# CarloLucibello/GraphNeuralNetworks.jl

Measured on AMD Instinct MI355X. Metric: edges/sec (fwd) GCNConv+GATConv, ogbn-products-shape; achieved HBM GB/s vs peak, higher is better.
Workload: dtype f32; 1 GPU; products-shape power-law graph N=2449029 E=61859140 (+N self loops, E'=64308169), D=100: GCNConv(100=>100,relu) fwd + GATConv(100=>16,heads=8,relu) fwd per step; edges counted = 2*E' per GPU; parallelism=replicas x1 (independent feature batches, no collective)

## Files before the change

graphneuralnetworks.jl_amd/csrc/plan.hip:

```cpp
#include <cstring>
#include <algorithm>
#include <vector>

#include "common.h"
#include "launch.h"
#include "pool.h"
#include "scratch.h"
#include "sort_scan.h"

namespace gnnmp {

int ensure_workspace(gnnmp_graph *p, size_t floats) { return grow(p->ws, p->ws_floats, floats, "hipMalloc(plan workspace)"); }

int ensure_arrive(gnnmp_graph *p, size_t n, size_t floats, hipStream_t stream) {
    GNNMP_TRY(grow(p->spart, p->spart_floats, floats, "hipMalloc(plan slice partials)"));
    if (n <= p->arrive_n) return GNNMP_OK;
    GNNMP_TRY(grow(p->arrive, p->arrive_n, n, "hipMalloc(plan arrival counters)"));
    const hipError_t e = hipMemsetAsync(p->arrive, 0, sizeof(uint32_t) * n, stream);
    if (e != hipSuccess) {
        p->arrive_n = 0;
        return hip_fail(e, "hipMemsetAsync(plan arrival counters)");
    }
    return GNNMP_OK;
}
// ... 88 lines not shown
    if (!ok) *bad = 1;
    rowptr[i] = (uint32_t)(ok ? v : (i == n_dst ? E : 0));
}
__global__ void csc_col_kernel(const void *rowval, int idx_bytes, int base, int64_t E, int64_t n_src, int32_t *col, int32_t *eid, int *bad) {
    int64_t p = (int64_t)blockIdx.x * blockDim.x + threadIdx.x;
    if (p >= E) return;
    int64_t s = load_index(rowval, p, idx_bytes, base);
    if (s < 0 || s >= n_src) {
        *bad = 1;
        s = 0;
    }
    col[p] = (int32_t)s;
    eid[p] = (int32_t)(uint32_t)p;
}

__global__ void plan_long_rows(const uint32_t *rowptr, int64_t n_dst, int thresh, int64_t *list,
                               int cap, int *count, unsigned long long *maxdeg) {
    int64_t i = (int64_t)blockIdx.x * blockDim.x + threadIdx.x;
    if (i >= n_dst) return;
    const int64_t beg = rowptr[i], end = rowptr[i + 1];
    const int64_t len = end - beg;
    if (len > 0) atomicMax(maxdeg, (unsigned long long)len);
    if (len > thresh) {
        int pos = atomicAdd(count, 1);
        if (pos < cap) {
            list[3 * pos] = i;
            list[3 * pos + 1] = beg;
            list[3 * pos + 2] = end;
        }
    }
}
__global__ void widen_u32_kernel(const uint32_t *in, int64_t n, int64_t *out) {
    int64_t i = (int64_t)blockIdx.x * blockDim.x + threadIdx.x;
    if (i < n) out[i] = (int64_t)in[i];
}

__global__ void slot_gather_kernel(const int32_t *idx, const float *v, int64_t Etot, int64_t n_valid,
                                   float *out) {
    int64_t p = (int64_t)blockIdx.x * blockDim.x + threadIdx.x;
    if (p >= Etot) return;
    const int64_t k = (uint32_t)idx[p];
    out[p] = k < n_valid ? v[k] : 1.0f;
}

__global__ void self_loops_kernel(const void *src, const void *dst, int idx_bytes, int base,
// ... 47 lines not shown

static inline unsigned nblocks(int64_t n, int bs) { return (unsigned)((n + bs - 1) / bs); }

int plan_long_thresh(int64_t Etot) {
    if (knob(KNOB_LONG_ROW) > 0) return knob(KNOB_LONG_ROW);
    int th = GNNMP_MIN_LONG_ROW;
    while (th < GNNMP_LONG_ROW && (double)th < 4e-5 * (double)Etot) th <<= 1;
    return th;
}

static int plan_chunk_slots() {
    const int v = knob(KNOB_CHUNK_SLOTS);
    return v >= 16 ? v : 128;
}

int plan_build_long_rows(gnnmp_graph *p, hipStream_t stream) {
    const int64_t n_dst = p->n_dst, Etot = p->n_total;
    const int BS = 256;
    const int cap = (int)std::min<int64_t>(Etot / std::max(1, p->long_thresh) + 1, n_dst + 1);
    DevBuf<int64_t> long_tmp;
    DevBuf<int> flags;
    GNNMP_HIP(flags.alloc(4));
    GNNMP_HIP(hipMemsetAsync(flags.get(), 0, sizeof(int) * 4, stream));
    GNNMP_HIP(long_tmp.alloc(3 * (size_t)std::max(cap, 1)));
    if (n_dst > 0) {
        plan_long_rows<<<nblocks(n_dst, BS), BS, 0, stream>>>(p->rowptr, n_dst, p->long_thresh, long_tmp.get(), cap, flags.get(),
                                                              reinterpret_cast<unsigned long long *>(flags.get() + 2));
        GNNMP_HIP(hipGetLastError());
    }
    int meta[4] = {0, 0, 0, 0};
    GNNMP_HIP(hipMemcpyAsync(meta, flags.get(), sizeof(int) * 4, hipMemcpyDeviceToHost, stream));
    GNNMP_HIP(hipStreamSynchronize(stream));
    unsigned long long md;
    memcpy(&md, meta + 2, sizeof(md));
    p->max_degree = (int64_t)md;
    p->n_long = std::min(meta[0], cap);
    if (p->n_long == 0) return GNNMP_OK;
    struct Tri { int64_t row, beg, end; };
    std::vector<Tri> h((size_t)p->n_long);
    GNNMP_HIP(hipMemcpy(h.data(), long_tmp.get(), sizeof(Tri) * h.size(), hipMemcpyDeviceToHost));
    std::sort(h.begin(), h.end(), [](const Tri &a, const Tri &b) { return a.row < b.row; });
    std::vector<int32_t> rows, cptr, crow, clrow;
    std::vector<uint32_t> cbeg, cend;
    cptr.push_back(0);
    const int64_t clen = std::min<int64_t>(p->long_thresh, plan_chunk_slots());
    for (const Tri &t : h) {
        const int64_t len = t.end - t.beg;
        const int64_t nch = (len + clen - 1) / clen;
        const int64_t csz = (len + nch - 1) / nch;
        for (int64_t c = 0; c < nch; ++c) {
            crow.push_back((int32_t)t.row);
            clrow.push_back((int32_t)rows.size());
            cbeg.push_back((uint32_t)(t.beg + c * csz));
            cend.push_back((uint32_t)std::min(t.beg + (c + 1) * csz, t.end));
        }
        rows.push_back((int32_t)t.row);
        cptr.push_back((int32_t)crow.size());
    }
    if (crow.size() >= (size_t)INT32_MAX)
        return fail(GNNMP_EUNSUPPORTED, "plan_create: %zu chunks of split rows exceed the int32 chunk index", crow.size());
    p->n_chunks = (int)crow.size();
    auto upload = [&](auto *&dst, const auto &v) -> hipError_t {
        const size_t bytes = sizeof(v[0]) * v.size();
        const hipError_t e = alloc_into(dst, v.size());
        if (e != hipSuccess) return e;
        p->bytes += (int64_t)bytes;
        return hipMemcpy(dst, v.data(), bytes, hipMemcpyHostToDevice);
    };
    GNNMP_HIP(upload(p->long_rows, rows));
    GNNMP_HIP(upload(p->long_cptr, cptr));
    GNNMP_HIP(upload(p->chunk_row, crow));
    GNNMP_HIP(upload(p->chunk_lrow, clrow));
    GNNMP_HIP(upload(p->chunk_beg, cbeg));
    GNNMP_HIP(upload(p->chunk_end, cend));
    return GNNMP_OK;
}

}

using namespace gnnmp;

extern "C" {

int gnnmp_plan_destroy(gnnmp_graph_t *p) { return plan_dispose(p, nullptr, false); }

int gnnmp_plan_reset_counters(gnnmp_graph_t *p, gnnmp_stream_t stream_) {
    hipStream_t stream = (hipStream_t)stream_;
    if (!p) return fail(GNNMP_EINVAL, "plan_reset_counters: null plan");
    if (p->arrive && p->arrive_n) GNNMP_HIP(hipMemsetAsync(p->arrive, 0, sizeof(uint32_t) * p->arrive_n, stream));
    if (p->ticket) GNNMP_HIP(hipMemsetAsync(p->ticket, 0, 2 * sizeof(uint32_t), stream));
// ... 67 lines not shown
    const int64_t Etot = n_edges + (add_self_loops ? n_dst : 0);
    if (Etot >= (int64_t)GNNMP_MAX_SLOTS || n_src >= (int64_t)INT32_MAX || n_dst >= (int64_t)INT32_MAX)
        return fail(GNNMP_EUNSUPPORTED, "plan_create: E' = %lld (limit 2^32 - 65536) / N = %lld (limit 2^31 - 2) exceed the plan format",
                    (long long)Etot, (long long)std::max(n_src, n_dst));

    PlanPtr p(new gnnmp_graph_t());
    p->n_src = n_src;
    p->n_dst = n_dst;
    p->n_edges = n_edges;
    p->n_total = Etot;
    p->self_loops = add_self_loops ? 1 : 0;
    p->long_thresh = plan_long_thresh(Etot);

    const int BS = 256;
    const size_t epad = (size_t)std::max<int64_t>(Etot, 1);
    DevBuf<int> flags;
    DevBuf<unsigned char> sort_keys;
    uint32_t *keys_out = nullptr;
    GNNMP_HIP(alloc_into(p->rowptr, (size_t)(n_dst + 1)));
    GNNMP_HIP(alloc_into(p->col, epad));
    GNNMP_HIP(alloc_into(p->eid, epad));
    GNNMP_HIP(flags.alloc(4));
    GNNMP_HIP(hipMemsetAsync(flags.get(), 0, sizeof(int) * 4, stream));
    p->bytes = (int64_t)(sizeof(int32_t) * ((size_t)(n_dst + 1) + 2 * epad));

    if (Etot > 0) {
        const size_t piece = (sizeof(uint32_t) * epad + 255) & ~(size_t)255;
        GNNMP_HIP(sort_keys.alloc(3 * piece));
        uint32_t *keys_in = reinterpret_cast<uint32_t *>(sort_keys.get());
        keys_out = reinterpret_cast<uint32_t *>(sort_keys.get() + piece);
        uint32_t *vals_in = reinterpret_cast<uint32_t *>(sort_keys.get() + 2 * piece);
        plan_fill_keys<<<nblocks(Etot, BS), BS, 0, stream>>>(src, dst, idx_bytes, index_base,
                                                             n_edges, Etot, n_src, n_dst, keys_in,
                                                             vals_in, flags.get());
        GNNMP_HIP(hipGetLastError());
        if (validate) {
            int bad = 0;
            GNNMP_HIP(hipMemcpyAsync(&bad, flags.get(), sizeof(int), hipMemcpyDeviceToHost, stream));
            GNNMP_HIP(hipStreamSynchronize(stream));
            if (bad)
                return fail(GNNMP_EBOUNDS, "plan_create: edge index outside 1..N (n_src=%lld n_dst=%lld)",
                            (long long)n_src, (long long)n_dst);
        }
        unsigned bits = 1;
        while (bits < 32 && ((int64_t)1 << bits) < n_dst) ++bits;
        GNNMP_TRY(radix_sort_pairs_u32(keys_in, keys_out, vals_in, reinterpret_cast<uint32_t *>(p->eid), (size_t)Etot, 0, (int)bits,
                                       stream));
        plan_col<<<nblocks(Etot, BS), BS, 0, stream>>>(src, idx_bytes, index_base, n_edges, Etot,
                                                       reinterpret_cast<uint32_t *>(p->eid), p->col);
        GNNMP_HIP(hipGetLastError());
    }
    plan_rowptr<<<nblocks(n_dst + 1, BS), BS, 0, stream>>>(keys_out, Etot, n_dst, p->rowptr);
    GNNMP_HIP(hipGetLastError());

    GNNMP_TRY(plan_build_long_rows(p.get(), stream));
    *out = p.release();
    return GNNMP_OK;
}

int gnnmp_plan_from_csc(gnnmp_graph_t **out, const void *colptr, const void *rowval, int idx_bytes, int index_base, int64_t n_src,
                        int64_t n_dst, int64_t n_edges, int validate, gnnmp_stream_t stream_) {
    hipStream_t stream = (hipStream_t)stream_;
    if (!out) return fail(GNNMP_EINVAL, "plan_from_csc: out is NULL");
    *out = nullptr;
    if (idx_bytes != 4 && idx_bytes != 8) return fail(GNNMP_EINVAL, "plan_from_csc: idx_bytes must be 4 or 8 (got %d)", idx_bytes);
    if (index_base != 0 && index_base != 1) return fail(GNNMP_EINVAL, "plan_from_csc: index_base must be 0 or 1 (got %d)", index_base);
    if (n_src < 0 || n_dst < 0 || n_edges < 0) return fail(GNNMP_EINVAL, "plan_from_csc: negative size");
    if (!colptr || (n_edges > 0 && !rowval)) return fail(GNNMP_EINVAL, "plan_from_csc: null colptr / rowval");
    if (n_edges >= (int64_t)GNNMP_MAX_SLOTS || n_src >= (int64_t)INT32_MAX || n_dst >= (int64_t)INT32_MAX)
        return fail(GNNMP_EUNSUPPORTED, "plan_from_csc: E = %lld (limit 2^32 - 65536) / N = %lld (limit 2^31 - 2) exceed the plan format",
                    (long long)n_edges, (long long)std::max(n_src, n_dst));
    PlanPtr p(new gnnmp_graph_t());
    p->n_src = n_src;
    p->n_dst = n_dst;
    p->n_edges = n_edges;
    p->n_total = n_edges;
    p->long_thresh = plan_long_thresh(n_edges);
    const int BS = 256;
    const size_t epad = (size_t)std::max<int64_t>(n_edges, 1);
    DevBuf<int> flags;
    GNNMP_HIP(alloc_into(p->rowptr, (size_t)(n_dst + 1)));
    GNNMP_HIP(alloc_into(p->col, epad));
    GNNMP_HIP(alloc_into(p->eid, epad));
    GNNMP_HIP(flags.alloc(4));
    GNNMP_HIP(hipMemsetAsync(flags.get(), 0, sizeof(int) * 4, stream));
    p->bytes = (int64_t)(sizeof(int32_t) * ((size_t)(n_dst + 1) + 2 * epad));
    csc_rowptr_kernel<<<nblocks(n_dst + 1, BS), BS, 0, stream>>>(colptr, idx_bytes, index_base, n_dst, n_edges, p->rowptr, flags.get());
    GNNMP_HIP(hipGetLastError());
    if (n_edges > 0) {
        csc_col_kernel<<<nblocks(n_edges, BS), BS, 0, stream>>>(rowval, idx_bytes, index_base, n_edges, n_src, p->col, p->eid, flags.get());
        GNNMP_HIP(hipGetLastError());
    }
    (void)validate;
    int bad = 0;
    GNNMP_HIP(hipMemcpyAsync(&bad, flags.get(), sizeof(int), hipMemcpyDeviceToHost, stream));
    GNNMP_HIP(hipStreamSynchronize(stream));
    if (bad)
        return fail(GNNMP_EBOUNDS, "plan_from_csc: colptr is not a monotone 0..E column pointer, or a row index lies outside 1..n_src "
                    "(n_src=%lld n_dst=%lld E=%lld)", (long long)n_src, (long long)n_dst, (long long)n_edges);
    GNNMP_TRY(plan_build_long_rows(p.get(), stream));
    *out = p.release();
    return GNNMP_OK;
}

int gnnmp_plan_slot_gather_f32(gnnmp_graph_t *p, int by, const float *v, float *out_slot,
                               gnnmp_stream_t stream_) {
    hipStream_t stream = (hipStream_t)stream_;
    if (!p) return fail(GNNMP_EINVAL, "plan_slot_gather: null plan");
    if (by != 0 && by != 1) return fail(GNNMP_EINVAL, "plan_slot_gather: `by` must be 0 (node) or 1 (edge)");
    if (p->n_total == 0) return GNNMP_OK;
    if (!v || !out_slot) return fail(GNNMP_EINVAL, "plan_slot_gather: null pointer");
    if (by == 0)
        slot_gather_kernel<<<nblocks(p->n_total, 256), 256, 0, stream>>>(p->col, v, p->n_total, p->n_src, out_slot);
    else
        slot_gather_kernel<<<nblocks(p->n_total, 256), 256, 0, stream>>>(p->eid, v, p->n_total, p->n_edges, out_slot);
// ... 94 lines not shown
```

graphneuralnetworks.jl_amd/csrc/plan_edit.hip:

```cpp
#include <algorithm>

#include "common.h"
#include "launch.h"
#include "pool.h"
#include "sort_scan.h"

namespace gnnmp {
namespace {

constexpr int BS = 256;
inline unsigned nblk(int64_t n) { return (unsigned)std::max<int64_t>(1, (n + BS - 1) / BS); }
inline size_t up64(size_t n) { return (n + 63) & ~(size_t)63; }

struct PoolScratch {
    void *p = nullptr;
    size_t cap = 0;
    hipStream_t stream;
    explicit PoolScratch(hipStream_t s) : stream(s) {}
    PoolScratch(const PoolScratch &) = delete;
    PoolScratch &operator=(const PoolScratch &) = delete;
    ~PoolScratch() { pool_park(p, cap, stream, true); }
    bool take(size_t bytes) { return pool_take(&p, &cap, std::max<size_t>(bytes, 256), stream); }
};

__device__ __forceinline__ int64_t row_of_slot(const uint32_t *__restrict__ rowptr, int64_t n_rows, int64_t p) {
    int64_t lo = 0, hi = n_rows;
    while (hi - lo > 1) {
        const int64_t mid = (lo + hi) >> 1;
        if ((int64_t)rowptr[mid] <= p) lo = mid; else hi = mid;
    }
    return lo;
}

enum { META_NKEEP = 0, META_EKEEP = 1, META_SLOTS = 2, META_MAXDEG = 3, META_BAD = 4, META_WORDS = 8 };

__global__ void __launch_bounds__(BS) rm_mark_kernel(int64_t N, int random, int none, DropArgs d, uint32_t *__restrict__ keep) {
    const int64_t i = (int64_t)blockIdx.x * BS + threadIdx.x;
    if (i > N) return;
// ... 344 lines not shown
```

graphneuralnetworks.jl_amd/csrc/pool.h:

```cpp
#pragma once
#include <hip/hip_runtime.h>
#include <stddef.h>

namespace gnnmp {
bool pool_take(void **out, size_t *cap, size_t bytes, hipStream_t stream);
void pool_park(void *p, size_t cap, hipStream_t stream, bool stream_known);
int pool_pick(const size_t *caps, int n, size_t bytes);
void pool_trim();
}
```

graphneuralnetworks.jl_amd/csrc/pool.hip:

```cpp
#include <mutex>

#include "pool.h"
#include "common.h"

namespace gnnmp {
namespace {
struct Parked {
    void *p = nullptr;
    size_t cap = 0;
    hipStream_t stream = nullptr;
    hipEvent_t ev = nullptr;
};
constexpr int POOL_SLOTS = 8;
struct DevicePool {
    Parked slots[POOL_SLOTS];
    hipEvent_t free_events[POOL_SLOTS] = {};
    int n_free_events = 0;
};
DevicePool g_pools[GNNMP_MAX_DEVICES];
std::mutex g_lock;

hipEvent_t event_get(DevicePool &dp) {
    if (dp.n_free_events > 0) return dp.free_events[--dp.n_free_events];
    hipEvent_t e = nullptr;
    if (hipEventCreateWithFlags(&e, hipEventDisableTiming) != hipSuccess) return nullptr;
    return e;
}
void event_put(DevicePool &dp, hipEvent_t e) {
    if (!e) return;
    if (dp.n_free_events < POOL_SLOTS) dp.free_events[dp.n_free_events++] = e;
    else (void)hipEventDestroy(e);
}
bool same_stream(hipStream_t a, hipStream_t b) { return a == b && a != hipStreamPerThread; }
}

int pool_pick(const size_t *caps, int n, size_t bytes) {
    int best = -1;
    for (int i = 0; i < n; ++i)
        if (caps[i] && caps[i] >= bytes && (best < 0 || caps[i] < caps[best])) best = i;
    if (best >= 0 && caps[best] <= 2 * bytes + (1 << 20)) return best;
    return -1;
}

bool pool_take(void **out, size_t *cap, size_t bytes, hipStream_t stream) {
    DevicePool &dp = g_pools[current_device()];
    Parked got;
    {
        std::lock_guard<std::mutex> lk(g_lock);
        size_t caps[POOL_SLOTS];
        for (int i = 0; i < POOL_SLOTS; ++i) caps[i] = dp.slots[i].p ? dp.slots[i].cap : 0;
        const int best = pool_pick(caps, POOL_SLOTS, bytes);
        if (best >= 0) {
            got = dp.slots[best];
            dp.slots[best] = Parked();
        }
    }
    if (got.p) {
        bool ok = true;
        if (!got.ev) {
            ok = hipDeviceSynchronize() == hipSuccess;
// ... 1 lines not shown
            if (!same_stream(got.stream, stream)) ok = hipStreamWaitEvent(stream, got.ev, 0) == hipSuccess;
            std::lock_guard<std::mutex> lk(g_lock);
            event_put(dp, got.ev);
        }
        if (ok) {
            *out = got.p;
            *cap = got.cap;
            return true;
        }
        (void)hipFree(got.p);
    }
    *cap = bytes;
    return hipMalloc(out, bytes) == hipSuccess;
}

void pool_park(void *p, size_t cap, hipStream_t stream, bool stream_known) {
    if (!p) return;
    int dev = current_device();
    {
        hipPointerAttribute_t at;
        if (hipPointerGetAttributes(&at, p) == hipSuccess && at.device >= 0 && at.device < GNNMP_MAX_DEVICES) {
            if (at.device != dev) stream_known = false;
            dev = at.device;
        } else {
            (void)hipGetLastError();
        }
    }
    DevicePool &dp = g_pools[dev];
    Parked in;
    in.p = p;
    in.cap = cap;
    Parked evict;
    {
        std::lock_guard<std::mutex> lk(g_lock);
        if (stream_known) {
            in.stream = stream;
            in.ev = event_get(dp);
            if (in.ev && hipEventRecord(in.ev, stream) != hipSuccess) {
                (void)hipGetLastError();
                event_put(dp, in.ev);
                in.ev = nullptr;
            }
        }
// ... 6 lines not shown
                if (dp.slots[i].cap < dp.slots[slot].cap) slot = i;
            if (dp.slots[slot].cap >= cap) {
                evict = in;
                in = Parked();
            } else {
                evict = dp.slots[slot];
            }
        }
        if (in.p) dp.slots[slot] = in;
        if (evict.ev) { event_put(dp, evict.ev); evict.ev = nullptr; }
    }
    if (evict.p) (void)hipFree(evict.p);
}

void pool_trim() {
    for (int d = 0; d < GNNMP_MAX_DEVICES; ++d) {
        Parked all[POOL_SLOTS];
        bool any = false;
        {
            std::lock_guard<std::mutex> lk(g_lock);
            DevicePool &dp = g_pools[d];
            for (int i = 0; i < POOL_SLOTS; ++i) {
                all[i] = dp.slots[i];
                dp.slots[i] = Parked();
                if (all[i].ev) event_put(dp, all[i].ev);
                any = any || all[i].p;
            }
        }
        if (!any) continue;
        for (int i = 0; i < POOL_SLOTS; ++i)
            if (all[i].p) (void)hipFree(all[i].p);
    }
}
}
```

graphneuralnetworks.jl_amd/csrc/sort_scan.h:

```cpp
#pragma once
#include <hip/hip_runtime.h>
#include <stddef.h>
#include <stdint.h>

namespace gnnmp {
int radix_sort_pairs_u32(const uint32_t *keys_in, uint32_t *keys_out, const uint32_t *vals_in, uint32_t *vals_out, size_t n,
                         int begin_bit, int end_bit, hipStream_t stream);
int radix_sort_keys_u64(const uint64_t *keys_in, uint64_t *keys_out, size_t n, int begin_bit, int end_bit, hipStream_t stream);
int radix_sort_pairs_u64(const uint64_t *keys_in, uint64_t *keys_out, const uint32_t *vals_in, uint32_t *vals_out, size_t n,
                         int begin_bit, int end_bit, hipStream_t stream);
size_t exclusive_scan_workspace(size_t n);
int exclusive_scan_i64(const int64_t *in, int64_t *out, size_t n, hipStream_t stream, int64_t *ws = nullptr);
int exclusive_scan_u32(const uint32_t *in, uint32_t *out, size_t n, hipStream_t stream, uint32_t *ws = nullptr);
}
```

graphneuralnetworks.jl_amd/csrc/sort_scan.hip:

```cpp
#include <algorithm>

#include "common.h"
#include "scratch.h"
#include "sort_scan.h"

namespace gnnmp {

constexpr int RS_WT = 2048;
constexpr int RS_WPB = 4;
constexpr int SC_CHUNK = 4096;

__device__ __forceinline__ void wave_lds_sync() {
    __builtin_amdgcn_fence(__ATOMIC_RELEASE, "wavefront");
    __builtin_amdgcn_wave_barrier();
    __builtin_amdgcn_fence(__ATOMIC_ACQUIRE, "wavefront");
}

template <class K>
__global__ void __launch_bounds__(64 * RS_WPB) rs_hist(const K *__restrict__ keys, size_t n, int shift, uint32_t *__restrict__ counts,
                                                       size_t n_tiles) {
    __shared__ uint32_t h[RS_WPB][256];
    const int lane = threadIdx.x & 63, w = threadIdx.x >> 6;
    const size_t tile = (size_t)blockIdx.x * RS_WPB + w;
    if (tile >= n_tiles) return;
// ... 220 lines not shown
int exclusive_scan_u32(const uint32_t *in, uint32_t *out, size_t n, hipStream_t stream, uint32_t *ws) {
    return exclusive_scan_impl<uint32_t>(in, out, n, stream, ws);
}

template <class K>
__global__ void __launch_bounds__(256) rs_varying_bits(const K *__restrict__ keys, size_t n, unsigned long long *__restrict__ out) {
    const K k0 = keys[0];
    unsigned long long v = 0;
    for (size_t i = (size_t)blockIdx.x * blockDim.x + threadIdx.x; i < n; i += (size_t)gridDim.x * blockDim.x)
        v |= (unsigned long long)(keys[i] ^ k0);
#pragma unroll
    for (int o = 32; o >= 1; o >>= 1) v |= __shfl_xor(v, o, 64);
    if ((threadIdx.x & 63) == 0 && v) atomicOr(out, v);
}

template <class K, bool PAIRS>
static int radix_sort_impl(const K *keys_in, K *keys_out, const uint32_t *vals_in, uint32_t *vals_out, size_t n, int begin_bit,
                           int end_bit, hipStream_t stream) {
    if (n == 0) return GNNMP_OK;
    if (n >= ((size_t)1 << 32)) return fail(GNNMP_EUNSUPPORTED, "radix sort: %zu elements exceed the 32-bit offset tables", n);
    const int passes = std::max(1, (end_bit - begin_bit + 7) / 8);
    const size_t n_tiles = (n + RS_WT - 1) / RS_WT;
    const size_t m = 256 * n_tiles;
    auto up = [](size_t b) { return (b + 255) & ~(size_t)255; };
    const size_t b_k = up(sizeof(K) * n), b_v = PAIRS ? up(sizeof(uint32_t) * n) : 0, b_c = up(sizeof(uint32_t) * m),
                 b_s = up(sizeof(uint32_t) * scan_blocks(m));
    DevBuf<unsigned char> arena;
    hipError_t e = arena.alloc(b_k + b_v + b_c + b_s + 256);
    if (e != hipSuccess) return hip_fail(e, "hipMalloc(radix sort temporaries)");
    K *ktmp = reinterpret_cast<K *>(arena.get());
    uint32_t *vtmp = PAIRS ? reinterpret_cast<uint32_t *>(arena.get() + b_k) : nullptr;
    uint32_t *counts = reinterpret_cast<uint32_t *>(arena.get() + b_k + b_v);
    uint32_t *sums = reinterpret_cast<uint32_t *>(arena.get() + b_k + b_v + b_c);
    unsigned long long *dvary = reinterpret_cast<unsigned long long *>(arena.get() + b_k + b_v + b_c + b_s), hvary = 0;
    const unsigned blocks = (unsigned)((n_tiles + RS_WPB - 1) / RS_WPB);
    const size_t scatter_lds = (size_t)RS_WT * RS_WPB * (sizeof(K) + (PAIRS ? sizeof(uint32_t) : 0)) + (256 * RS_WPB + 256) * sizeof(uint32_t);
    e = hipFuncSetAttribute(reinterpret_cast<const void *>(&rs_scatter<K, PAIRS>), hipFuncAttributeMaxDynamicSharedMemorySize,
                            (int)scatter_lds);
    if (e != hipSuccess) return hip_fail(e, "hipFuncSetAttribute(rs_scatter)");
    e = hipMemsetAsync(dvary, 0, sizeof(unsigned long long), stream);
    if (e == hipSuccess) {
        const unsigned vb = (unsigned)std::min<size_t>((n + 255) / 256, (size_t)device_cus() * 8);
        rs_varying_bits<K><<<vb, 256, 0, stream>>>(keys_in, n, dvary);
        e = hipMemcpyAsync(&hvary, dvary, sizeof(hvary), hipMemcpyDeviceToHost, stream);
    }
    if (e == hipSuccess) e = hipStreamSynchronize(stream);
    if (e != hipSuccess) return hip_fail(e, "radix sort: varying bits");
    const K *ksrc = keys_in;
    const uint32_t *vsrc = vals_in;
    for (int p = 0; p < passes; ++p) {
        const int shift = begin_bit + 8 * p;
        if (((hvary >> shift) & 255ull) == 0) continue;
        rs_hist<K><<<blocks, 64 * RS_WPB, 0, stream>>>(ksrc, n, shift, counts, n_tiles);
        exclusive_scan_enqueue<uint32_t>(counts, counts, m, sums, stream);
        K *kdst = (ksrc == keys_out) ? ktmp : keys_out;
        uint32_t *vdst = (ksrc == keys_out) ? vtmp : vals_out;
        rs_scatter<K, PAIRS><<<blocks, 64 * RS_WPB, scatter_lds, stream>>>(ksrc, vsrc, n, shift, counts, n_tiles, kdst, vdst);
        e = hipGetLastError();
        if (e != hipSuccess) return hip_fail(e, "radix sort pass");
        ksrc = kdst;
        vsrc = vdst;
    }
    if (ksrc != keys_out) {
        e = hipMemcpyAsync(keys_out, ksrc, sizeof(K) * n, hipMemcpyDeviceToDevice, stream);
        if (e == hipSuccess && PAIRS) e = hipMemcpyAsync(vals_out, vsrc, sizeof(uint32_t) * n, hipMemcpyDeviceToDevice, stream);
        if (e != hipSuccess) return hip_fail(e, "radix sort copy-out");
    }
    e = hipStreamSynchronize(stream);
    if (e != hipSuccess) return hip_fail(e, "radix sort");
    return GNNMP_OK;
}

int radix_sort_pairs_u32(const uint32_t *keys_in, uint32_t *keys_out, const uint32_t *vals_in, uint32_t *vals_out, size_t n,
                         int begin_bit, int end_bit, hipStream_t stream) {
    return radix_sort_impl<uint32_t, true>(keys_in, keys_out, vals_in, vals_out, n, begin_bit, end_bit, stream);
}
int radix_sort_keys_u64(const uint64_t *keys_in, uint64_t *keys_out, size_t n, int begin_bit, int end_bit, hipStream_t stream) {
    return radix_sort_impl<uint64_t, false>(keys_in, keys_out, nullptr, nullptr, n, begin_bit, end_bit, stream);
}
int radix_sort_pairs_u64(const uint64_t *keys_in, uint64_t *keys_out, const uint32_t *vals_in, uint32_t *vals_out, size_t n,
                         int begin_bit, int end_bit, hipStream_t stream) {
    return radix_sort_impl<uint64_t, true>(keys_in, keys_out, vals_in, vals_out, n, begin_bit, end_bit, stream);
}

}
```

Measured before the change: 12.92 billion edges/s.

## Build long-row chunk tables on device and drop plan-time host syncs

Long-row detection and chunk splitting move from a host-side sort and loop to a device pipeline: flag, scan, list, scan, fill. Plan scratch now comes from a pooled arena, and the radix sort gains a workspace variant that skips the varying-bits readback. The validation readback is deferred so it shares the single final sync. This targets plan-construction latency (host round trips, allocations, host-to-device uploads), not the per-step forward kernels, so the measured edges/s is likely unaffected unless plan build is timed.

New measurement: 12.92 billion edges/s, median of 2. No clear change (-0.0%).

```diff
diff --git a/graphneuralnetworks.jl_amd/csrc/plan.hip b/graphneuralnetworks.jl_amd/csrc/plan.hip
--- a/graphneuralnetworks.jl_amd/csrc/plan.hip
+++ b/graphneuralnetworks.jl_amd/csrc/plan.hip
@@ -1,9 +1,8 @@
-#include <cstring>
 #include <algorithm>
-#include <vector>
 
 #include "common.h"
 #include "launch.h"
+#include "plan_chunks.h"
 #include "pool.h"
 #include "scratch.h"
 #include "sort_scan.h"
@@ -126,21 +125,56 @@
     eid[p] = (int32_t)(uint32_t)p;
 }
 
-__global__ void plan_long_rows(const uint32_t *rowptr, int64_t n_dst, int thresh, int64_t *list,
-                               int cap, int *count, unsigned long long *maxdeg) {
-    int64_t i = (int64_t)blockIdx.x * blockDim.x + threadIdx.x;
-    if (i >= n_dst) return;
-    const int64_t beg = rowptr[i], end = rowptr[i + 1];
-    const int64_t len = end - beg;
-    if (len > 0) atomicMax(maxdeg, (unsigned long long)len);
-    if (len > thresh) {
-        int pos = atomicAdd(count, 1);
-        if (pos < cap) {
-            list[3 * pos] = i;
-            list[3 * pos + 1] = beg;
-            list[3 * pos + 2] = end;
-        }
-    }
+enum { META_BAD = 0, META_NLONG = 1, META_NCHUNKS = 2, META_MAXDEG = 3, META_WORDS = 4 };
+
+__global__ void __launch_bounds__(256) plan_long_flag(const uint32_t *__restrict__ rowptr, int64_t n_dst, int thresh,
+                                                      uint32_t *__restrict__ flag, uint32_t *__restrict__ meta) {
+    const int64_t i = (int64_t)blockIdx.x * 256 + threadIdx.x;
+    int64_t len = 0;
+    if (i < n_dst) len = (int64_t)rowptr[i + 1] - (int64_t)rowptr[i];
+    if (i <= n_dst) flag[i] = len > thresh ? 1u : 0u;
+    uint32_t m = len > 0 ? (uint32_t)len : 0u;
+#pragma unroll
+    for (int o = 32; o > 0; o >>= 1) m = max(m, (uint32_t)__shfl_xor(m, o, 64));
+    if ((threadIdx.x & 63) == 0 && m > 0) atomicMax(&meta[META_MAXDEG], m);
+}
+__global__ void __launch_bounds__(256) plan_long_list(const uint32_t *__restrict__ rowptr, int64_t n_dst, const uint32_t *__restrict__ flag,
+                                                      const uint32_t *__restrict__ lidx, int64_t clen, int cap,
+                                                      int32_t *__restrict__ long_rows, uint32_t *__restrict__ nch) {
+    const int64_t i = (int64_t)blockIdx.x * 256 + threadIdx.x;
+    if (i >= n_dst || !flag[i]) return;
+    const uint32_t r = lidx[i];
+    if (r >= (uint32_t)cap) return;
+    long_rows[r] = (int32_t)i;
+    nch[r] = (uint32_t)plan_row_chunks((int64_t)rowptr[i + 1] - (int64_t)rowptr[i], clen);
+}
+__global__ void __launch_bounds__(256) plan_chunk_fill(const uint32_t *__restrict__ rowptr, int64_t n_dst, const uint32_t *__restrict__ lidx,
+                                                       int cap, const int32_t *__restrict__ long_rows, const uint32_t *__restrict__ cptr,
+                                                       int64_t chunk_cap, int32_t *__restrict__ chunk_row, int32_t *__restrict__ chunk_lrow,
+                                                       uint32_t *__restrict__ chunk_beg, uint32_t *__restrict__ chunk_end,
+                                                       uint32_t *__restrict__ meta) {
+    const int64_t c = (int64_t)blockIdx.x * 256 + threadIdx.x;
+    const uint32_t n_long = min(lidx[n_dst], (uint32_t)cap);
+    const uint32_t n_chunks = cptr[n_long];
+    if (c == 0) {
+        meta[META_NLONG] = n_long;
+        meta[META_NCHUNKS] = n_chunks;
+    }
+    if (c >= (int64_t)n_chunks || c >= chunk_cap || n_long == 0) return;
+    uint32_t lo = 0, hi = n_long;
+    while (hi - lo > 1) {
+        const uint32_t mid = lo + ((hi - lo) >> 1);
+        if ((int64_t)cptr[mid] <= c) lo = mid; else hi = mid;
+    }
+    const int64_t row = long_rows[lo];
+    const int64_t nch = (int64_t)cptr[lo + 1] - (int64_t)cptr[lo];
+    if (row < 0 || row >= n_dst || nch < 1) return;
+    uint32_t b, e;
+    plan_chunk_range((int64_t)rowptr[row], (int64_t)rowptr[row + 1], nch, c - (int64_t)cptr[lo], &b, &e);
+    chunk_row[c] = (int32_t)row;
+    chunk_lrow[c] = (int32_t)lo;
+    chunk_beg[c] = b;
+    chunk_end[c] = e;
 }
 __global__ void widen_u32_kernel(const uint32_t *in, int64_t n, int64_t *out) {
     int64_t i = (int64_t)blockIdx.x * blockDim.x + threadIdx.x;
@@ -218,66 +252,105 @@
     return v >= 16 ? v : 128;
 }
 
-int plan_build_long_rows(gnnmp_graph *p, hipStream_t stream) {
-    const int64_t n_dst = p->n_dst, Etot = p->n_total;
+struct LongScratch {
+    int cap = 0;
+    int64_t clen = 0;
+    int64_t chunk_cap = 0;
+    size_t n_scan = 0;
+    size_t o_meta = 0, o_flag = 0, o_lidx = 0, o_scan = 0, o_nch = 0, o_rows = 0, o_cptr = 0, o_crow = 0, o_clrow = 0, o_cbeg = 0, o_cend = 0;
+    size_t bytes = 0;
+    LongScratch(int64_t n_dst, int64_t Etot, int thresh) {
+        cap = (int)std::min<int64_t>(Etot / std::max(1, thresh) + 1, n_dst + 1);
+        clen = std::max<int64_t>(1, std::min<int64_t>(thresh, plan_chunk_slots()));
+        chunk_cap = Etot / clen + cap;
+        n_scan = std::max(exclusive_scan_workspace((size_t)n_dst + 1), exclusive_scan_workspace((size_t)cap + 1));
+        auto piece = [this](size_t elems) {
+            const size_t o = bytes;
+            bytes += (sizeof(uint32_t) * elems + 255) & ~(size_t)255;
+            return o;
+        };
+        o_meta = piece(META_WORDS);
+        o_flag = piece((size_t)n_dst + 1);
+        o_lidx = piece((size_t)n_dst + 1);
+        o_scan = piece(n_scan);
+        o_nch = piece((size_t)cap + 1);
+        o_rows = piece((size_t)cap);
+        o_cptr = piece((size_t)cap + 1);
+        o_crow = piece((size_t)chunk_cap);
+        o_clrow = piece((size_t)chunk_cap);
+        o_cbeg = piece((size_t)chunk_cap);
+        o_cend = piece((size_t)chunk_cap);
+    }
+};
+template <class T>
+static inline T *piece_at(void *base, size_t off) { return reinterpret_cast<T *>(static_cast<unsigned char *>(base) + off); }
+
+static int long_scratch_check(const LongScratch &L) {
+    if (L.chunk_cap >= ((int64_t)1 << 32))
+        return fail(GNNMP_EUNSUPPORTED, "plan_create: up to %lld chunks of split rows exceed the 32-bit chunk tables", (long long)L.chunk_cap);
+    return GNNMP_OK;
+}
+static int build_long_rows_in(gnnmp_graph *p, hipStream_t stream, const LongScratch &L, void *base, uint32_t *bad) {
+    const int64_t n_dst = p->n_dst;
     const int BS = 256;
-    const int cap = (int)std::min<int64_t>(Etot / std::max(1, p->long_thresh) + 1, n_dst + 1);
-    DevBuf<int64_t> long_tmp;
-    DevBuf<int> flags;
-    GNNMP_HIP(flags.alloc(4));
-    GNNMP_HIP(hipMemsetAsync(flags.get(), 0, sizeof(int) * 4, stream));
-    GNNMP_HIP(long_tmp.alloc(3 * (size_t)std::max(cap, 1)));
+    uint32_t *const meta = piece_at<uint32_t>(base, L.o_meta), *const flag = piece_at<uint32_t>(base, L.o_flag),
+                   *const lidx = piece_at<uint32_t>(base, L.o_lidx), *const scan_ws = piece_at<uint32_t>(base, L.o_scan),
+                   *const nch = piece_at<uint32_t>(base, L.o_nch), *const cptr = piece_at<uint32_t>(base, L.o_cptr),
+                   *const cbeg = piece_at<uint32_t>(base, L.o_cbeg), *const cend = piece_at<uint32_t>(base, L.o_cend);
+    int32_t *const rows = piece_at<int32_t>(base, L.o_rows), *const crow = piece_at<int32_t>(base, L.o_crow),
+                  *const clrow = piece_at<int32_t>(base, L.o_clrow);
+    GNNMP_HIP(hipMemsetAsync(nch, 0, sizeof(uint32_t) * ((size_t)L.cap + 1), stream));
+    plan_long_flag<<<nblocks(n_dst + 1, BS), BS, 0, stream>>>(p->rowptr, n_dst, p->long_thresh, flag, meta);
+    GNNMP_HIP(hipGetLastError());
+    GNNMP_TRY(exclusive_scan_u32(flag, lidx, (size_t)n_dst + 1, stream, scan_ws));
     if (n_dst > 0) {
-        plan_long_rows<<<nblocks(n_dst, BS), BS, 0, stream>>>(p->rowptr, n_dst, p->long_thresh, long_tmp.get(), cap, flags.get(),
-                                                              reinterpret_cast<unsigned long long *>(flags.get() + 2));
+        plan_long_list<<<nblocks(n_dst, BS), BS, 0, stream>>>(p->rowptr, n_dst, flag, lidx, L.clen, L.cap, rows, nch);
         GNNMP_HIP(hipGetLastError());
     }
-    int meta[4] = {0, 0, 0, 0};
-    GNNMP_HIP(hipMemcpyAsync(meta, flags.get(), sizeof(int) * 4, hipMemcpyDeviceToHost, stream));
+    GNNMP_TRY(exclusive_scan_u32(nch, cptr, (size_t)L.cap + 1, stream, scan_ws));
+    plan_chunk_fill<<<nblocks(std::max<int64_t>(L.chunk_cap, 1), BS), BS, 0, stream>>>(p->rowptr, n_dst, lidx, L.cap, rows, cptr, L.chunk_cap,
+                                                                                      crow, clrow, cbeg, cend, meta);
+    GNNMP_HIP(hipGetLastError());
+    uint32_t h[META_WORDS] = {};
+    GNNMP_HIP(hipMemcpyAsync(h, meta, sizeof(h), hipMemcpyDeviceToHost, stream));
     GNNMP_HIP(hipStreamSynchronize(stream));
-    unsigned long long md;
-    memcpy(&md, meta + 2, sizeof(md));
-    p->max_degree = (int64_t)md;
-    p->n_long = std::min(meta[0], cap);
+    if (bad) {
+        *bad = h[META_BAD];
+        if (*bad) return GNNMP_OK;
+    }
+    p->max_degree = (int64_t)h[META_MAXDEG];
+    p->n_long = (int)std::min<uint32_t>(h[META_NLONG], (uint32_t)L.cap);
     if (p->n_long == 0) return GNNMP_OK;
-    struct Tri { int64_t row, beg, end; };
-    std::vector<Tri> h((size_t)p->n_long);
-    GNNMP_HIP(hipMemcpy(h.data(), long_tmp.get(), sizeof(Tri) * h.size(), hipMemcpyDeviceToHost));
-    std::sort(h.begin(), h.end(), [](const Tri &a, const Tri &b) { return a.row < b.row; });
-    std::vector<int32_t> rows, cptr, crow, clrow;
-    std::vector<uint32_t> cbeg, cend;
-    cptr.push_back(0);
-    const int64_t clen = std::min<int64_t>(p->long_thresh, plan_chunk_slots());
-    for (const Tri &t : h) {
-        const int64_t len = t.end - t.beg;
-        const int64_t nch = (len + clen - 1) / clen;
-        const int64_t csz = (len + nch - 1) / nch;
-        for (int64_t c = 0; c < nch; ++c) {
-            crow.push_back((int32_t)t.row);
-            clrow.push_back((int32_t)rows.size());
-            cbeg.push_back((uint32_t)(t.beg + c * csz));
-            cend.push_back((uint32_t)std::min(t.beg + (c + 1) * csz, t.end));
-        }
-        rows.push_back((int32_t)t.row);
-        cptr.push_back((int32_t)crow.size());
-    }
-    if (crow.size() >= (size_t)INT32_MAX)
-        return fail(GNNMP_EUNSUPPORTED, "plan_create: %zu chunks of split rows exceed the int32 chunk index", crow.size());
-    p->n_chunks = (int)crow.size();
-    auto upload = [&](auto *&dst, const auto &v) -> hipError_t {
-        const size_t bytes = sizeof(v[0]) * v.size();
-        const hipError_t e = alloc_into(dst, v.size());
+    const size_t n_long = (size_t)p->n_long, n_chunks = (size_t)h[META_NCHUNKS];
+    if (n_chunks >= (size_t)INT32_MAX)
+        return fail(GNNMP_EUNSUPPORTED, "plan_create: %zu chunks of split rows exceed the int32 chunk index", n_chunks);
+    if ((int64_t)n_chunks > L.chunk_cap)
+        return fail(GNNMP_EINVAL, "plan_create: %zu chunks of split rows for a bound of %lld: rowptr is not monotone", n_chunks,
+                    (long long)L.chunk_cap);
+    p->n_chunks = (int)n_chunks;
+    auto keep = [&](auto *&dst, const void *src, size_t n) -> hipError_t {
+        const size_t bytes = sizeof(*dst) * n;
+        const hipError_t e = alloc_into(dst, n);
         if (e != hipSuccess) return e;
         p->bytes += (int64_t)bytes;
-        return hipMemcpy(dst, v.data(), bytes, hipMemcpyHostToDevice);
+        return hipMemcpyAsync(dst, src, bytes, hipMemcpyDeviceToDevice, stream);
     };
-    GNNMP_HIP(upload(p->long_rows, rows));
-    GNNMP_HIP(upload(p->long_cptr, cptr));
-    GNNMP_HIP(upload(p->chunk_row, crow));
-    GNNMP_HIP(upload(p->chunk_lrow, clrow));
-    GNNMP_HIP(upload(p->chunk_beg, cbeg));
-    GNNMP_HIP(upload(p->chunk_end, cend));
-    return GNNMP_OK;
+    GNNMP_HIP(keep(p->long_rows, rows, n_long));
+    GNNMP_HIP(keep(p->long_cptr, cptr, n_long + 1));
+    GNNMP_HIP(keep(p->chunk_row, crow, n_chunks));
+    GNNMP_HIP(keep(p->chunk_lrow, clrow, n_chunks));
+    GNNMP_HIP(keep(p->chunk_beg, cbeg, n_chunks));
+    GNNMP_HIP(keep(p->chunk_end, cend, n_chunks));
+    return GNNMP_OK;
+}
+
+int plan_build_long_rows(gnnmp_graph *p, hipStream_t stream) {
+    const LongScratch L(p->n_dst, p->n_total, p->long_thresh);
+    GNNMP_TRY(long_scratch_check(L));
+    PoolScratch sc(stream);
+    if (!sc.take(L.bytes)) return fail(GNNMP_EALLOC, "plan build: hipMalloc of %zu bytes of scratch failed", L.bytes);
+    GNNMP_HIP(hipMemsetAsync(piece_at<uint32_t>(sc.p, L.o_meta), 0, sizeof(uint32_t) * META_WORDS, stream));
+    return build_long_rows_in(p, stream, L, sc.p, nullptr);
 }
 
 }
@@ -375,46 +448,50 @@
 
     const int BS = 256;
     const size_t epad = (size_t)std::max<int64_t>(Etot, 1);
-    DevBuf<int> flags;
-    DevBuf<unsigned char> sort_keys;
+    const LongScratch L(n_dst, Etot, p->long_thresh);
+    GNNMP_TRY(long_scratch_check(L));
+    const size_t piece = Etot > 0 ? (sizeof(uint32_t) * epad + 255) & ~(size_t)255 : 0;
+    const size_t sort_ws = Etot > 0 ? radix_sort_pairs_u32_workspace((size_t)Etot) : 0;
+    PoolScratch sc(stream);
+    if (!sc.take(3 * piece + sort_ws + L.bytes))
+        return fail(GNNMP_EALLOC, "plan_create: hipMalloc of %zu bytes of scratch failed", 3 * piece + sort_ws + L.bytes);
+    unsigned char *const sbase = static_cast<unsigned char *>(sc.p);
+    void *const lbase = sbase + 3 * piece + sort_ws;
+    uint32_t *const meta = piece_at<uint32_t>(lbase, L.o_meta);
     uint32_t *keys_out = nullptr;
-    GNNMP_HIP(alloc_into(p->rowptr, (size_t)(n_dst + 1)));
-    GNNMP_HIP(alloc_into(p->col, epad));
-    GNNMP_HIP(alloc_into(p->eid, epad));
-    GNNMP_HIP(flags.alloc(4));
-    GNNMP_HIP(hipMemsetAsync(flags.get(), 0, sizeof(int) * 4, stream));
+    GNNMP_HIP(hipMemsetAsync(meta, 0, sizeof(uint32_t) * META_WORDS, stream));
     p->bytes = (int64_t)(sizeof(int32_t) * ((size_t)(n_dst + 1) + 2 * epad));
 
     if (Etot > 0) {
-        const size_t piece = (sizeof(uint32_t) * epad + 255) & ~(size_t)255;
-        GNNMP_HIP(sort_keys.alloc(3 * piece));
-        uint32_t *keys_in = reinterpret_cast<uint32_t *>(sort_keys.get());
-        keys_out = reinterpret_cast<uint32_t *>(sort_keys.get() + piece);
-        uint32_t *vals_in = reinterpret_cast<uint32_t *>(sort_keys.get() + 2 * piece);
+        uint32_t *keys_in = reinterpret_cast<uint32_t *>(sbase);
+        keys_out = reinterpret_cast<uint32_t *>(sbase + piece);
+        uint32_t *vals_in = reinterpret_cast<uint32_t *>(sbase + 2 * piece);
         plan_fill_keys<<<nblocks(Etot, BS), BS, 0, stream>>>(src, dst, idx_bytes, index_base,
                                                              n_edges, Etot, n_src, n_dst, keys_in,
-                                                             vals_in, flags.get());
+                                                             vals_in, reinterpret_cast<int *>(meta + META_BAD));
         GNNMP_HIP(hipGetLastError());
-        if (validate) {
-            int bad = 0;
-            GNNMP_HIP(hipMemcpyAsync(&bad, flags.get(), sizeof(int), hipMemcpyDeviceToHost, stream));
-            GNNMP_HIP(hipStreamSynchronize(stream));
-            if (bad)
-                return fail(GNNMP_EBOUNDS, "plan_create: edge index outside 1..N (n_src=%lld n_dst=%lld)",
-                            (long long)n_src, (long long)n_dst);
-        }
+        GNNMP_HIP(alloc_into(p->eid, epad));
         unsigned bits = 1;
         while (bits < 32 && ((int64_t)1 << bits) < n_dst) ++bits;
-        GNNMP_TRY(radix_sort_pairs_u32(keys_in, keys_out, vals_in, reinterpret_cast<uint32_t *>(p->eid), (size_t)Etot, 0, (int)bits,
-                                       stream));
+        GNNMP_TRY(radix_sort_pairs_u32_ws(keys_in, keys_out, vals_in, reinterpret_cast<uint32_t *>(p->eid), (size_t)Etot, 0, (int)bits,
+                                          sbase + 3 * piece, sort_ws, ~(uint64_t)0, stream));
+        GNNMP_HIP(alloc_into(p->col, epad));
         plan_col<<<nblocks(Etot, BS), BS, 0, stream>>>(src, idx_bytes, index_base, n_edges, Etot,
                                                        reinterpret_cast<uint32_t *>(p->eid), p->col);
         GNNMP_HIP(hipGetLastError());
-    }
+    } else {
+        GNNMP_HIP(alloc_into(p->eid, epad));
+        GNNMP_HIP(alloc_into(p->col, epad));
+    }
+    GNNMP_HIP(alloc_into(p->rowptr, (size_t)(n_dst + 1)));
     plan_rowptr<<<nblocks(n_dst + 1, BS), BS, 0, stream>>>(keys_out, Etot, n_dst, p->rowptr);
     GNNMP_HIP(hipGetLastError());
 
-    GNNMP_TRY(plan_build_long_rows(p.get(), stream));
+    uint32_t bad = 0;
+    GNNMP_TRY(build_long_rows_in(p.get(), stream, L, lbase, validate ? &bad : nullptr));
+    if (bad)
+        return fail(GNNMP_EBOUNDS, "plan_create: edge index outside 1..N (n_src=%lld n_dst=%lld)",
+                    (long long)n_src, (long long)n_dst);
     *out = p.release();
     return GNNMP_OK;
 }
@@ -439,27 +516,29 @@
     p->long_thresh = plan_long_thresh(n_edges);
     const int BS = 256;
     const size_t epad = (size_t)std::max<int64_t>(n_edges, 1);
-    DevBuf<int> flags;
+    const LongScratch L(n_dst, n_edges, p->long_thresh);
+    GNNMP_TRY(long_scratch_check(L));
+    PoolScratch sc(stream);
+    if (!sc.take(L.bytes)) return fail(GNNMP_EALLOC, "plan_from_csc: hipMalloc of %zu bytes of scratch failed", L.bytes);
+    uint32_t *const meta = piece_at<uint32_t>(sc.p, L.o_meta);
+    int *const flags = reinterpret_cast<int *>(meta + META_BAD);
     GNNMP_HIP(alloc_into(p->rowptr, (size_t)(n_dst + 1)));
     GNNMP_HIP(alloc_into(p->col, epad));
     GNNMP_HIP(alloc_into(p->eid, epad));
-    GNNMP_HIP(flags.alloc(4));
-    GNNMP_HIP(hipMemsetAsync(flags.get(), 0, sizeof(int) * 4, stream));
+    GNNMP_HIP(hipMemsetAsync(meta, 0, sizeof(uint32_t) * META_WORDS, stream));
     p->bytes = (int64_t)(sizeof(int32_t) * ((size_t)(n_dst + 1) + 2 * epad));
-    csc_rowptr_kernel<<<nblocks(n_dst + 1, BS), BS, 0, stream>>>(colptr, idx_bytes, index_base, n_dst, n_edges, p->rowptr, flags.get());
+    csc_rowptr_kernel<<<nblocks(n_dst + 1, BS), BS, 0, stream>>>(colptr, idx_bytes, index_base, n_dst, n_edges, p->rowptr, flags);
     GNNMP_HIP(hipGetLastError());
     if (n_edges > 0) {
-        csc_col_kernel<<<nblocks(n_edges, BS), BS, 0, stream>>>(rowval, idx_bytes, index_base, n_edges, n_src, p->col, p->eid, flags.get());
+        csc_col_kernel<<<nblocks(n_edges, BS), BS, 0, stream>>>(rowval, idx_bytes, index_base, n_edges, n_src, p->col, p->eid, flags);
         GNNMP_HIP(hipGetLastError());
     }
     (void)validate;
-    int bad = 0;
-    GNNMP_HIP(hipMemcpyAsync(&bad, flags.get(), sizeof(int), hipMemcpyDeviceToHost, stream));
-    GNNMP_HIP(hipStreamSynchronize(stream));
+    uint32_t bad = 0;
+    GNNMP_TRY(build_long_rows_in(p.get(), stream, L, sc.p, &bad));
     if (bad)
         return fail(GNNMP_EBOUNDS, "plan_from_csc: colptr is not a monotone 0..E column pointer, or a row index lies outside 1..n_src "
                     "(n_src=%lld n_dst=%lld E=%lld)", (long long)n_src, (long long)n_dst, (long long)n_edges);
-    GNNMP_TRY(plan_build_long_rows(p.get(), stream));
     *out = p.release();
     return GNNMP_OK;
 }
diff --git a/graphneuralnetworks.jl_amd/csrc/plan_chunks.h b/graphneuralnetworks.jl_amd/csrc/plan_chunks.h
--- /dev/null
+++ b/graphneuralnetworks.jl_amd/csrc/plan_chunks.h
@@ -0,0 +1,19 @@
+#pragma once
+#include <stdint.h>
+
+#if defined(__HIPCC__) || defined(__CUDACC__)
+#define GNNMP_CHUNKS_HD __host__ __device__
+#else
+#define GNNMP_CHUNKS_HD
+#endif
+
+namespace gnnmp {
+GNNMP_CHUNKS_HD inline int64_t plan_row_chunks(int64_t len, int64_t clen) { return (len + clen - 1) / clen; }
+GNNMP_CHUNKS_HD inline int64_t plan_chunk_size(int64_t len, int64_t nch) { return (len + nch - 1) / nch; }
+GNNMP_CHUNKS_HD inline void plan_chunk_range(int64_t beg, int64_t end, int64_t nch, int64_t c, uint32_t *cbeg, uint32_t *cend) {
+    const int64_t csz = plan_chunk_size(end - beg, nch);
+    const int64_t e = beg + (c + 1) * csz;
+    *cbeg = (uint32_t)(beg + c * csz);
+    *cend = (uint32_t)(e < end ? e : end);
+}
+}
diff --git a/graphneuralnetworks.jl_amd/csrc/plan_edit.hip b/graphneuralnetworks.jl_amd/csrc/plan_edit.hip
--- a/graphneuralnetworks.jl_amd/csrc/plan_edit.hip
+++ b/graphneuralnetworks.jl_amd/csrc/plan_edit.hip
@@ -11,17 +11,6 @@
 constexpr int BS = 256;
 inline unsigned nblk(int64_t n) { return (unsigned)std::max<int64_t>(1, (n + BS - 1) / BS); }
 inline size_t up64(size_t n) { return (n + 63) & ~(size_t)63; }
-
-struct PoolScratch {
-    void *p = nullptr;
-    size_t cap = 0;
-    hipStream_t stream;
-    explicit PoolScratch(hipStream_t s) : stream(s) {}
-    PoolScratch(const PoolScratch &) = delete;
-    PoolScratch &operator=(const PoolScratch &) = delete;
-    ~PoolScratch() { pool_park(p, cap, stream, true); }
-    bool take(size_t bytes) { return pool_take(&p, &cap, std::max<size_t>(bytes, 256), stream); }
-};
 
 __device__ __forceinline__ int64_t row_of_slot(const uint32_t *__restrict__ rowptr, int64_t n_rows, int64_t p) {
     int64_t lo = 0, hi = n_rows;
diff --git a/graphneuralnetworks.jl_amd/csrc/pool.h b/graphneuralnetworks.jl_amd/csrc/pool.h
--- a/graphneuralnetworks.jl_amd/csrc/pool.h
+++ b/graphneuralnetworks.jl_amd/csrc/pool.h
@@ -3,8 +3,26 @@
 #include <stddef.h>
 
 namespace gnnmp {
-bool pool_take(void **out, size_t *cap, size_t bytes, hipStream_t stream);
-void pool_park(void *p, size_t cap, hipStream_t stream, bool stream_known);
+enum PoolKind { POOL_OBJECTS = 0, POOL_SCRATCH = 1 };
+bool pool_take(void **out, size_t *cap, size_t bytes, hipStream_t stream, PoolKind kind = POOL_OBJECTS);
+void pool_park(void *p, size_t cap, hipStream_t stream, bool stream_known, PoolKind kind = POOL_OBJECTS);
 int pool_pick(const size_t *caps, int n, size_t bytes);
 void pool_trim();
+
+#pragma GCC visibility push(hidden)
+constexpr size_t POOL_SCRATCH_KEEP_MAX = (size_t)4 << 30;
+struct PoolScratch {
+    void *p = nullptr;
+    size_t cap = 0;
+    hipStream_t stream;
+    explicit PoolScratch(hipStream_t s) : stream(s) {}
+    PoolScratch(const PoolScratch &) = delete;
+    PoolScratch &operator=(const PoolScratch &) = delete;
+    ~PoolScratch() {
+        if (cap <= POOL_SCRATCH_KEEP_MAX) pool_park(p, cap, stream, true, POOL_SCRATCH);
+        else if (p) (void)hipFree(p);
+    }
+    bool take(size_t bytes) { return pool_take(&p, &cap, bytes < 256 ? 256 : bytes, stream, POOL_SCRATCH); }
+};
+#pragma GCC visibility pop
 }
diff --git a/graphneuralnetworks.jl_amd/csrc/pool.hip b/graphneuralnetworks.jl_amd/csrc/pool.hip
--- a/graphneuralnetworks.jl_amd/csrc/pool.hip
+++ b/graphneuralnetworks.jl_amd/csrc/pool.hip
@@ -17,7 +17,7 @@
     hipEvent_t free_events[POOL_SLOTS] = {};
     int n_free_events = 0;
 };
-DevicePool g_pools[GNNMP_MAX_DEVICES];
+DevicePool g_pools[GNNMP_MAX_DEVICES][2];
 std::mutex g_lock;
 
 hipEvent_t event_get(DevicePool &dp) {
@@ -42,8 +42,8 @@
     return -1;
 }
 
-bool pool_take(void **out, size_t *cap, size_t bytes, hipStream_t stream) {
-    DevicePool &dp = g_pools[current_device()];
+bool pool_take(void **out, size_t *cap, size_t bytes, hipStream_t stream, PoolKind kind) {
+    DevicePool &dp = g_pools[current_device()][kind];
     Parked got;
     {
         std::lock_guard<std::mutex> lk(g_lock);
@@ -75,7 +75,7 @@
     return hipMalloc(out, bytes) == hipSuccess;
 }
 
-void pool_park(void *p, size_t cap, hipStream_t stream, bool stream_known) {
+void pool_park(void *p, size_t cap, hipStream_t stream, bool stream_known, PoolKind kind) {
     if (!p) return;
     int dev = current_device();
     {
@@ -87,7 +87,7 @@
             (void)hipGetLastError();
         }
     }
-    DevicePool &dp = g_pools[dev];
+    DevicePool &dp = g_pools[dev][kind];
     Parked in;
     in.p = p;
     in.cap = cap;
@@ -124,12 +124,12 @@
 }
 
 void pool_trim() {
-    for (int d = 0; d < GNNMP_MAX_DEVICES; ++d) {
+    for (int d = 0; d < 2 * GNNMP_MAX_DEVICES; ++d) {
         Parked all[POOL_SLOTS];
         bool any = false;
         {
             std::lock_guard<std::mutex> lk(g_lock);
-            DevicePool &dp = g_pools[d];
+            DevicePool &dp = g_pools[d >> 1][d & 1];
             for (int i = 0; i < POOL_SLOTS; ++i) {
                 all[i] = dp.slots[i];
                 dp.slots[i] = Parked();
diff --git a/graphneuralnetworks.jl_amd/csrc/sort_scan.h b/graphneuralnetworks.jl_amd/csrc/sort_scan.h
--- a/graphneuralnetworks.jl_amd/csrc/sort_scan.h
+++ b/graphneuralnetworks.jl_amd/csrc/sort_scan.h
@@ -9,6 +9,9 @@
 int radix_sort_keys_u64(const uint64_t *keys_in, uint64_t *keys_out, size_t n, int begin_bit, int end_bit, hipStream_t stream);
 int radix_sort_pairs_u64(const uint64_t *keys_in, uint64_t *keys_out, const uint32_t *vals_in, uint32_t *vals_out, size_t n,
                          int begin_bit, int end_bit, hipStream_t stream);
+size_t radix_sort_pairs_u32_workspace(size_t n);
+int radix_sort_pairs_u32_ws(const uint32_t *keys_in, uint32_t *keys_out, const uint32_t *vals_in, uint32_t *vals_out, size_t n,
+                            int begin_bit, int end_bit, void *ws, size_t ws_bytes, uint64_t vary_mask, hipStream_t stream);
 size_t exclusive_scan_workspace(size_t n);
 int exclusive_scan_i64(const int64_t *in, int64_t *out, size_t n, hipStream_t stream, int64_t *ws = nullptr);
 int exclusive_scan_u32(const uint32_t *in, uint32_t *out, size_t n, hipStream_t stream, uint32_t *ws = nullptr);
diff --git a/graphneuralnetworks.jl_amd/csrc/sort_scan.hip b/graphneuralnetworks.jl_amd/csrc/sort_scan.hip
--- a/graphneuralnetworks.jl_amd/csrc/sort_scan.hip
+++ b/graphneuralnetworks.jl_amd/csrc/sort_scan.hip
@@ -258,43 +258,40 @@
     if ((threadIdx.x & 63) == 0 && v) atomicOr(out, v);
 }
 
+static inline size_t rs_up(size_t b) { return (b + 255) & ~(size_t)255; }
 template <class K, bool PAIRS>
-static int radix_sort_impl(const K *keys_in, K *keys_out, const uint32_t *vals_in, uint32_t *vals_out, size_t n, int begin_bit,
-                           int end_bit, hipStream_t stream) {
+static size_t radix_sort_ws_bytes(size_t n) {
+    const size_t m = 256 * ((n + RS_WT - 1) / RS_WT);
+    return rs_up(sizeof(K) * n) + (PAIRS ? rs_up(sizeof(uint32_t) * n) : 0) + rs_up(sizeof(uint32_t) * m) +
+           rs_up(sizeof(uint32_t) * scan_blocks(m));
+}
+
+template <class K, bool PAIRS>
+static int radix_sort_enqueue(const K *keys_in, K *keys_out, const uint32_t *vals_in, uint32_t *vals_out, size_t n, int begin_bit,
+                              int end_bit, void *ws, size_t ws_bytes, uint64_t vary_mask, hipStream_t stream) {
     if (n == 0) return GNNMP_OK;
     if (n >= ((size_t)1 << 32)) return fail(GNNMP_EUNSUPPORTED, "radix sort: %zu elements exceed the 32-bit offset tables", n);
+    if (!ws || (reinterpret_cast<uintptr_t>(ws) & 255) != 0 || ws_bytes < radix_sort_ws_bytes<K, PAIRS>(n))
+        return fail(GNNMP_EINVAL, "radix sort: workspace of %zu bytes (need %zu, 256-byte aligned)", ws_bytes, radix_sort_ws_bytes<K, PAIRS>(n));
     const int passes = std::max(1, (end_bit - begin_bit + 7) / 8);
     const size_t n_tiles = (n + RS_WT - 1) / RS_WT;
     const size_t m = 256 * n_tiles;
-    auto up = [](size_t b) { return (b + 255) & ~(size_t)255; };
-    const size_t b_k = up(sizeof(K) * n), b_v = PAIRS ? up(sizeof(uint32_t) * n) : 0, b_c = up(sizeof(uint32_t) * m),
-                 b_s = up(sizeof(uint32_t) * scan_blocks(m));
-    DevBuf<unsigned char> arena;
-    hipError_t e = arena.alloc(b_k + b_v + b_c + b_s + 256);
-    if (e != hipSuccess) return hip_fail(e, "hipMalloc(radix sort temporaries)");
-    K *ktmp = reinterpret_cast<K *>(arena.get());
-    uint32_t *vtmp = PAIRS ? reinterpret_cast<uint32_t *>(arena.get() + b_k) : nullptr;
-    uint32_t *counts = reinterpret_cast<uint32_t *>(arena.get() + b_k + b_v);
-    uint32_t *sums = reinterpret_cast<uint32_t *>(arena.get() + b_k + b_v + b_c);
-    unsigned long long *dvary = reinterpret_cast<unsigned long long *>(arena.get() + b_k + b_v + b_c + b_s), hvary = 0;
+    const size_t b_k = rs_up(sizeof(K) * n), b_v = PAIRS ? rs_up(sizeof(uint32_t) * n) : 0, b_c = rs_up(sizeof(uint32_t) * m);
+    unsigned char *const base = static_cast<unsigned char *>(ws);
+    K *ktmp = reinterpret_cast<K *>(base);
+    uint32_t *vtmp = PAIRS ? reinterpret_cast<uint32_t *>(base + b_k) : nullptr;
+    uint32_t *counts = reinterpret_cast<uint32_t *>(base + b_k + b_v);
+    uint32_t *sums = reinterpret_cast<uint32_t *>(base + b_k + b_v + b_c);
     const unsigned blocks = (unsigned)((n_tiles + RS_WPB - 1) / RS_WPB);
     const size_t scatter_lds = (size_t)RS_WT * RS_WPB * (sizeof(K) + (PAIRS ? sizeof(uint32_t) : 0)) + (256 * RS_WPB + 256) * sizeof(uint32_t);
-    e = hipFuncSetAttribute(reinterpret_cast<const void *>(&rs_scatter<K, PAIRS>), hipFuncAttributeMaxDynamicSharedMemorySize,
-                            (int)scatter_lds);
+    hipError_t e = hipFuncSetAttribute(reinterpret_cast<const void *>(&rs_scatter<K, PAIRS>), hipFuncAttributeMaxDynamicSharedMemorySize,
+                                       (int)scatter_lds);
     if (e != hipSuccess) return hip_fail(e, "hipFuncSetAttribute(rs_scatter)");
-    e = hipMemsetAsync(dvary, 0, sizeof(unsigned long long), stream);
-    if (e == hipSuccess) {
-        const unsigned vb = (unsigned)std::min<size_t>((n + 255) / 256, (size_t)device_cus() * 8);
-        rs_varying_bits<K><<<vb, 256, 0, stream>>>(keys_in, n, dvary);
-        e = hipMemcpyAsync(&hvary, dvary, sizeof(hvary), hipMemcpyDeviceToHost, stream);
-    }
-    if (e == hipSuccess) e = hipStreamSynchronize(stream);
-    if (e != hipSuccess) return hip_fail(e, "radix sort: varying bits");
     const K *ksrc = keys_in;
     const uint32_t *vsrc = vals_in;
     for (int p = 0; p < passes; ++p) {
         const int shift = begin_bit + 8 * p;
-        if (((hvary >> shift) & 255ull) == 0) continue;
+        if (((vary_mask >> shift) & 255ull) == 0) continue;
         rs_hist<K><<<blocks, 64 * RS_WPB, 0, stream>>>(ksrc, n, shift, counts, n_tiles);
         exclusive_scan_enqueue<uint32_t>(counts, counts, m, sums, stream);
         K *kdst = (ksrc == keys_out) ? ktmp : keys_out;
@@ -310,11 +307,39 @@
         if (e == hipSuccess && PAIRS) e = hipMemcpyAsync(vals_out, vsrc, sizeof(uint32_t) * n, hipMemcpyDeviceToDevice, stream);
         if (e != hipSuccess) return hip_fail(e, "radix sort copy-out");
     }
+    return GNNMP_OK;
+}
+
+template <class K, bool PAIRS>
+static int radix_sort_impl(const K *keys_in, K *keys_out, const uint32_t *vals_in, uint32_t *vals_out, size_t n, int begin_bit,
+                           int end_bit, hipStream_t stream) {
+    if (n == 0) return GNNMP_OK;
+    if (n >= ((size_t)1 << 32)) return fail(GNNMP_EUNSUPPORTED, "radix sort: %zu elements exceed the 32-bit offset tables", n);
+    const size_t ws_bytes = radix_sort_ws_bytes<K, PAIRS>(n);
+    DevBuf<unsigned char> arena;
+    hipError_t e = arena.alloc(ws_bytes + 256);
+    if (e != hipSuccess) return hip_fail(e, "hipMalloc(radix sort temporaries)");
+    unsigned long long *dvary = reinterpret_cast<unsigned long long *>(arena.get() + ws_bytes), hvary = 0;
+    e = hipMemsetAsync(dvary, 0, sizeof(unsigned long long), stream);
+    if (e == hipSuccess) {
+        const unsigned vb = (unsigned)std::min<size_t>((n + 255) / 256, (size_t)device_cus() * 8);
+        rs_varying_bits<K><<<vb, 256, 0, stream>>>(keys_in, n, dvary);
+        e = hipMemcpyAsync(&hvary, dvary, sizeof(hvary), hipMemcpyDeviceToHost, stream);
+    }
+    if (e == hipSuccess) e = hipStreamSynchronize(stream);
+    if (e != hipSuccess) return hip_fail(e, "radix sort: varying bits");
+    GNNMP_TRY((radix_sort_enqueue<K, PAIRS>(keys_in, keys_out, vals_in, vals_out, n, begin_bit, end_bit, arena.get(), ws_bytes,
+                                            (uint64_t)hvary, stream)));
     e = hipStreamSynchronize(stream);
     if (e != hipSuccess) return hip_fail(e, "radix sort");
     return GNNMP_OK;
 }
 
+size_t radix_sort_pairs_u32_workspace(size_t n) { return radix_sort_ws_bytes<uint32_t, true>(n); }
+int radix_sort_pairs_u32_ws(const uint32_t *keys_in, uint32_t *keys_out, const uint32_t *vals_in, uint32_t *vals_out, size_t n,
+                            int begin_bit, int end_bit, void *ws, size_t ws_bytes, uint64_t vary_mask, hipStream_t stream) {
+    return radix_sort_enqueue<uint32_t, true>(keys_in, keys_out, vals_in, vals_out, n, begin_bit, end_bit, ws, ws_bytes, vary_mask, stream);
+}
 int radix_sort_pairs_u32(const uint32_t *keys_in, uint32_t *keys_out, const uint32_t *vals_in, uint32_t *vals_out, size_t n,
                          int begin_bit, int end_bit, hipStream_t stream) {
     return radix_sort_impl<uint32_t, true>(keys_in, keys_out, vals_in, vals_out, n, begin_bit, end_bit, stream);
```
